# yichuan-w/LEANN

Hardware: AMD Instinct MI355X
Metric: queries/sec at recall@10>=0.9, 1M-chunk HNSW, MiniLM-L6 recompute (higher is better)
Workload: dtype fp16

## Files before the change

leann_amd/csrc/lm_attn_v2.hip:

```cpp
#include <hip/hip_fp16.h>

#include <cstdlib>

#include "lm_internal.h"

namespace lm {

typedef _Float16 half8 __attribute__((ext_vector_type(8)));
typedef _Float16 half4 __attribute__((ext_vector_type(4)));
typedef _Float16 half2v __attribute__((ext_vector_type(2)));
typedef float float16v __attribute__((ext_vector_type(16)));
typedef float float2v __attribute__((ext_vector_type(2)));

template <int NT, int HD = 32>
__global__ __launch_bounds__(256) void k_attn_varlen_hd32_v2(const __half* __restrict__ qkv, const int32_t* __restrict__ cu,
                                                             __half* __restrict__ out, int heads, float scale_log2e, int n_units) {
    extern __shared__ __align__(16) unsigned char smem[];
    const int per = gridDim.x >> 3;
    const int unit = n_units < 0 ? (int)blockIdx.x : (int)((blockIdx.x & 7) * per + (blockIdx.x >> 3));
    if (unit >= (n_units < 0 ? -n_units : n_units)) return;
    const int seq = unit / heads, h = unit % heads;
    const int tok0 = cu[seq];
    const int len = cu[seq + 1] - tok0;
    constexpr int A2_HD = HD, A2_KSTRIDE = HD + 8, PARTS = HD / 8, KS = HD / 16, DT = HD / 32;
// ... 151 lines not shown
                }
        }
    }
}

}

#ifndef LM_HOST_EMULATION
template <int HD>
static int attn_v2_launch_hd(const void* d_qkv, const int32_t* d_cu_seqlens, int32_t n_seqs, int32_t heads, int32_t max_len, void* d_out,
                             void* stream) {
    using namespace lm;
    if constexpr (HD == 32) {
        const char* gen = getenv("LEANN_MI355X_ATTN");
        const char* var = getenv("LEANN_MI355X_ATTN3");
        if (!(gen && gen[0] == '2') && !(var && var[0] == '9')) return lm_attn_v3_launch_hd32(d_qkv, d_cu_seqlens, n_seqs, heads, max_len, d_out, 0, stream);
    }
    const int nt = (max_len + 31) / 32;
    const size_t shmem = ((size_t)32 * nt * (HD + 8) + (size_t)HD * (32 * nt + 4)) * 2;
    const float scale_log2e = 1.4426950408889634f / sqrtf((float)HD);
    const char* xo = getenv("LEANN_MI355X_ATTN_XCD");
    const int n_units = (xo && xo[0] == '0') ? -(n_seqs * heads) : n_seqs * heads;
    dim3 grid((unsigned)((n_seqs * heads + 7) / 8 * 8)), block(256);
    hipStream_t st = (hipStream_t)stream;
    const __half* q = (const __half*)d_qkv;
    __half* o = (__half*)d_out;
    kt_attn_work(d_cu_seqlens, n_seqs, heads * HD, stream);
    KtScope kt(LM_KT_ATTN, stream, 0.0);
    switch (nt) {
#define CASEA(n)                                                                                                                         \
    case n: {                                                                                                                            \
// ... 46 lines not shown
```

leann_amd/csrc/lm_attn_v3.hip:

```cpp
#include <hip/hip_fp16.h>

#include <algorithm>
#include <cstdlib>

#include "lm_h384_stream.h"

namespace lm {

typedef _Float16 half2v __attribute__((ext_vector_type(2)));

__device__ __forceinline__ half4 a3_lds_read_tr16(const unsigned char* p) {
#ifdef LM_EMULATED_DEVICE
    return emul::ds_read_tr16_b64<half4>(p);
#else
    typedef __fp16 fp16x4 __attribute__((__vector_size__(4 * sizeof(__fp16))));
    typedef __attribute__((address_space(3))) fp16x4 lds_fp16x4;
    return __builtin_bit_cast(half4, __builtin_amdgcn_ds_read_tr16_b64_v4f16((lds_fp16x4*)p));
#endif
}

#if defined(LM_DIAG) && !defined(LM_EMULATED_DEVICE)
constexpr int A3_STAMP_WAVES = 1 << 17, A3_STAMP_WORDS = 12;
__device__ unsigned long long g_a3_stamps[A3_STAMP_WAVES * A3_STAMP_WORDS];
#define A3_STAMPS 1
#define A3_NOW() ((VAR & 4) ? __builtin_amdgcn_s_memtime() : 0ull)
#else
#define A3_STAMPS 0
#define A3_NOW() 0ull
#endif

__device__ __forceinline__ float a3_max3(float a, float b, float c) { return __builtin_fmaxf(__builtin_fmaxf(a, b), c); }
__device__ __forceinline__ float a3_max(float a, float b) { return __builtin_fmaxf(a, b); }

constexpr float A3_THR = 8.0f;

template <int NT, int VAR>
__global__ __launch_bounds__(256, 4) void k_attn_varlen_hd32_v3(const __half* __restrict__ qkv, const int32_t* __restrict__ cu,
                                                                __half* __restrict__ out, int heads, float scale_log2e, int n_units, int64_t hm_tokens) {
    extern __shared__ __align__(16) unsigned char smem[];
    const int per = gridDim.x >> 3;
    const int unit = n_units < 0 ? (int)blockIdx.x : (int)((blockIdx.x & 7) * per + (blockIdx.x >> 3));
    if (unit >= (n_units < 0 ? -n_units : n_units)) return;
    const int seq = unit / heads, h = unit - seq * heads;
    const int tok0 = cu[seq];
    const int len = cu[seq + 1] - tok0;
    if (len <= 0) return;
    [[maybe_unused]] const unsigned long long ts0 = A3_NOW();
    const int H = heads * 32;
    const int rsb = hm_tokens ? 64 : 6 * H;
    constexpr int Tp = 32 * NT;
    unsigned char* Ks = smem;
// ... 13 lines not shown
            const int j = wv + 4 * i;
            if (j < 2 * nt) {
                const int row = 16 * j + rl;
                const int rowc = row < len ? row : len - 1;
                const unsigned ro = (unsigned)(rowc * rsb);
                lm_dma16_sv(kbase, ro + (unsigned)((pos ^ ((row >> 2) & 3)) << 4), Ks + 1024 * j);
                lm_dma16_sv(vbase, ro + (unsigned)(pos << 4), Vs + 1024 * j);
            }
        }
    }
    half8 qraw[2][2];
#pragma unroll
    for (int qi = 0; qi < 2; ++qi) {
        const int qrow = 32 * (wv + 4 * qi) + r31;
        const unsigned char* qp = base + (int64_t)(qrow < len ? qrow : len - 1) * rsb + g * 16;
        const half8 z = {0, 0, 0, 0, 0, 0, 0, 0};
        const half8 q0 = *(const half8*)qp, q1 = *(const half8*)(qp + 32);
        qraw[qi][0] = qrow < len ? q0 : z;
        qraw[qi][1] = qrow < len ? q1 : z;
    }
    [[maybe_unused]] const unsigned long long ts1 = A3_NOW();
    T4_WAIT_VM(0);
    [[maybe_unused]] const unsigned long long ts2 = A3_NOW();
    __syncthreads();
    [[maybe_unused]] const unsigned long long ts3 = A3_NOW();
    [[maybe_unused]] unsigned long long tacc_setup = 0, tacc_loop = 0, tacc_epi = 0, nqb_done = 0;

    const int sw = (r31 >> 2) & 3;
    const unsigned char* kf0 = Ks + r31 * 64 + ((g ^ sw) << 4);
    const unsigned char* kf1 = Ks + r31 * 64 + (((2 + g) ^ sw) << 4);
    const unsigned char* vf = Vs + g * 256 + ((lane >> 2) & 3) * 64 + ((lane >> 4) & 1) * 32 + (lane & 3) * 8;
    const int tail = len & 31;
    const float lenv = (float)(tail - 4 * g);

#pragma unroll
    for (int qi = 0; qi < 2; ++qi) {
        const int qb = wv + 4 * qi;
        if (qb >= nt) break;
        const int qrow = 32 * qb + r31;
        [[maybe_unused]] const unsigned long long tq0 = A3_NOW();
        half8 qf0, qf1;
#pragma unroll
        for (int e = 0; e < 8; ++e) {
            qf0[e] = (_Float16)((float)qraw[qi][0][e] * scale_log2e);
            qf1[e] = (_Float16)((float)qraw[qi][1][e] * scale_log2e);
        }
        float16v cm, o;
#pragma unroll
        for (int r = 0; r < 16; ++r) {
            cm[r] = 0.f;
            o[r] = 0.f;
        }
        float2v l2 = {0.f, 0.f}, l2b = {0.f, 0.f};

        float16v s;
        {
            const half8 k0 = *(const half8*)kf0, k1 = *(const half8*)kf1;
            s = __builtin_amdgcn_mfma_f32_32x32x16_f16(k0, qf0, cm, 0, 0, 0);
            s = __builtin_amdgcn_mfma_f32_32x32x16_f16(k1, qf1, s, 0, 0, 0);
        }
        [[maybe_unused]] const unsigned long long tq1 = A3_NOW();
        for (int t = 0; t < nt; ++t) {
            const bool more = t + 1 < nt;
            if (t > 0) {
                const half8 k0 = *(const half8*)(kf0 + 2048 * t), k1 = *(const half8*)(kf1 + 2048 * t);
                s = __builtin_amdgcn_mfma_f32_32x32x16_f16(k0, qf0, cm, 0, 0, 0);
                s = __builtin_amdgcn_mfma_f32_32x32x16_f16(k1, qf1, s, 0, 0, 0);
            }
            const unsigned char* vt = vf + 2048 * t;
            const half4 va0 = a3_lds_read_tr16(vt), vb0 = a3_lds_read_tr16(vt + 512), va1 = a3_lds_read_tr16(vt + 1024), vb1 = a3_lds_read_tr16(vt + 1536);
            if (!more && tail) {
                float lb = (lenv - 0.5f) * 1.0e30f;
                LM_KEEP_LOCAL(lb);
#pragma unroll
                for (int r = 0; r < 16; ++r) s[r] = __builtin_amdgcn_fmed3f(s[r], lb - (float)((r & 3) + 8 * (r >> 2)) * 1.0e30f, -3.0e38f);
            }
            float tm;
            {
                const float m0 = a3_max3(s[0], s[1], s[2]), m1 = a3_max3(s[3], s[4], s[5]), m2 = a3_max3(s[6], s[7], s[8]);
                const float m3 = a3_max3(s[9], s[10], s[11]), m4 = a3_max3(s[12], s[13], s[14]);
                tm = a3_max(a3_max3(m0, m1, m2), a3_max3(m3, m4, s[15]));
                uint32_t a = __builtin_bit_cast(uint32_t, tm), b = a;
                lane32_swap(a, b);
                tm = a3_max(__builtin_bit_cast(float, a), __builtin_bit_cast(float, b));
            }
            const bool first = t == 0;
            if (first || __ballot(tm > A3_THR) != 0) {
                const float delta = first ? tm : fmaxf(tm, 0.f);
                if (!first) {
                    const float alpha = __builtin_amdgcn_exp2f(-delta);
#pragma unroll
                    for (int r = 0; r < 16; ++r) o[r] *= alpha;
                    l2 *= (float2v){alpha, alpha};
                    l2b *= (float2v){alpha, alpha};
                }
                const float2v d2 = {delta, delta};
#pragma unroll
                for (int r = 0; r < 16; r += 2) {
                    const float2v a = (float2v){s[r], s[r + 1]} - d2, b = (float2v){cm[r], cm[r + 1]} - d2;
                    s[r] = a[0];
                    s[r + 1] = a[1];
                    cm[r] = b[0];
                    cm[r + 1] = b[1];
                }
            }
            half8 p0, p1;
#pragma unroll
            for (int r = 0; r < 8; r += 2) {
                const float2v e0 = {__builtin_amdgcn_exp2f(s[r]), __builtin_amdgcn_exp2f(s[r + 1])};
                const float2v e1 = {__builtin_amdgcn_exp2f(s[8 + r]), __builtin_amdgcn_exp2f(s[9 + r])};
                l2 += e0;
                l2b += e1;
                p0[r] = (_Float16)e0[0];
                p0[r + 1] = (_Float16)e0[1];
                p1[r] = (_Float16)e1[0];
                p1[r + 1] = (_Float16)e1[1];
            }
            const half8 v0 = {va0[0], va0[1], va0[2], va0[3], vb0[0], vb0[1], vb0[2], vb0[3]};
            const half8 v1 = {va1[0], va1[1], va1[2], va1[3], vb1[0], vb1[1], vb1[2], vb1[3]};
            o = __builtin_amdgcn_mfma_f32_32x32x16_f16(v0, p0, o, 0, 0, 0);
            o = __builtin_amdgcn_mfma_f32_32x32x16_f16(v1, p1, o, 0, 0, 0);
        }
        [[maybe_unused]] const unsigned long long tq2 = A3_NOW();
        float l = (l2[0] + l2[1]) + (l2b[0] + l2b[1]);
        {
            uint32_t a = __builtin_bit_cast(uint32_t, l), b = a;
            lane32_swap(a, b);
            l = __builtin_bit_cast(float, a) + __builtin_bit_cast(float, b);
        }
        const float inv = 1.0f / l;
        if (qrow < len) {
            _Float16* orow = (_Float16*)out + (int64_t)(tok0 + qrow) * H + h * 32;
#pragma unroll
            for (int r4 = 0; r4 < 4; ++r4) {
                const float2v i2 = {inv, inv};
                const float2v a = (float2v){o[4 * r4], o[4 * r4 + 1]} * i2, b = (float2v){o[4 * r4 + 2], o[4 * r4 + 3]} * i2;
                const half4 w = {(_Float16)a[0], (_Float16)a[1], (_Float16)b[0], (_Float16)b[1]};
// ... 36 lines not shown
#if defined(LM_DIAG) && !defined(LM_HOST_EMULATION) && !defined(LM_EMULATED_DEVICE)
extern "C" int lm_attn_v3_stamps_read(unsigned long long* out, int64_t max_words, int reset) {
    const size_t total = (size_t)lm::A3_STAMP_WAVES * lm::A3_STAMP_WORDS;
    const size_t n = std::min<size_t>(total, (size_t)max_words);
    if (hipMemcpyFromSymbol(out, HIP_SYMBOL(lm::g_a3_stamps), n * sizeof(unsigned long long)) != hipSuccess) return LM_EHIP;
    if (reset) {
        void* p = nullptr;
        if (hipGetSymbolAddress(&p, HIP_SYMBOL(lm::g_a3_stamps)) != hipSuccess || hipMemset(p, 0, total * sizeof(unsigned long long)) != hipSuccess) return LM_EHIP;
    }
    return LM_OK;
}
#endif

#ifndef LM_HOST_EMULATION
int lm_attn_v3_launch_hd32(const void* d_qkv, const int32_t* d_cu_seqlens, int32_t n_seqs, int32_t heads, int32_t max_len, void* d_out, int64_t total_tokens,
                           void* stream) {
    using namespace lm;
    const int nt = (max_len + 31) / 32;
    const size_t shmem = (size_t)32 * nt * 128;
    const float scale_log2e = 1.4426950408889634f / sqrtf(32.0f);
    const char* xo = getenv("LEANN_MI355X_ATTN_XCD");
    const int n_units = (xo && xo[0] == '0') ? -(n_seqs * heads) : n_seqs * heads;
    dim3 grid((unsigned)((n_seqs * heads + 7) / 8 * 8)), block(256);
    hipStream_t st = (hipStream_t)stream;
    const __half* q = (const __half*)d_qkv;
    __half* o = (__half*)d_out;
    kt_attn_work(d_cu_seqlens, n_seqs, heads * 32, stream);
    KtScope kt(LM_KT_ATTN, stream, 0.0);
    int var = 0;
#if A3_STAMPS
    const char* ve = getenv("LEANN_MI355X_ATTN3");
    if (ve && ve[0] == '4') var = 4;
#define A3_CASE4(n) CASEV(n, 4);
#else
#define A3_CASE4(n)
#endif
    switch (nt * 8 + var) {
#define CASEV(n, v) \
    case n * 8 + v: hipLaunchKernelGGL((k_attn_varlen_hd32_v3<n, v>), grid, block, shmem, st, q, d_cu_seqlens, o, heads, scale_log2e, n_units, total_tokens); break
#define CASEA(n) CASEV(n, 0); A3_CASE4(n)
        CASEA(1); CASEA(2); CASEA(3); CASEA(4); CASEA(5); CASEA(6); CASEA(7); CASEA(8);
#undef CASEA
#undef CASEV
#undef A3_CASE4
        default: LM_FAIL(LM_EINVAL, "lm_attn_varlen_hd32_f16 supports sequence lengths 1..256");
    }
    LM_HIP(hipGetLastError());
    return LM_OK;
}
#endif
```

leann_amd/csrc/lm_encoder_forward.cpp:

```cpp
#include <algorithm>
#include <cstdint>
#include <cstdlib>
#include <string>

#include "lm_internal.h"

static int64_t small_tokens_limit() {
    const char* e = getenv("LEANN_MI355X_SMALL_TOKENS");
    return e ? (int64_t)atoll(e) : (int64_t)LM_BERT_SMALL_TOKENS;
}

lm::H384FirstHalf lm::h384_first_half_form(int32_t heads, int32_t max_len, int64_t total_tokens, int32_t n_seqs) {
    auto is = [](const char* name, char c) {
        const char* e = getenv(name);
        return e && e[0] == c;
    };
    if (heads != 12 || max_len > 256) return H384_PAIR_ROW_MAJOR;
    if (is("LEANN_MI355X_QKV_LAYOUT", '0') || is("LEANN_MI355X_ATTN3", '9') || is("LEANN_MI355X_ATTN", '2')) return H384_PAIR_ROW_MAJOR;
    if (is("LEANN_MI355X_FUSED_QKV_ATTN", '0')) return H384_PAIR_HEAD_MAJOR;
    if (is("LEANN_MI355X_FUSED_QKV_ATTN", '1')) return H384_FUSED;
    return n_seqs > 0 && total_tokens >= (int64_t)H384_FUSED_MIN_MEAN_LEN * n_seqs ? H384_FUSED : H384_PAIR_HEAD_MAJOR;
}
extern "C" int lm_h384_first_half_form(int32_t heads, int32_t max_len, int64_t total_tokens, int32_t n_seqs) {
    return (int)lm::h384_first_half_form(heads, max_len, total_tokens, n_seqs);
// ... 9 lines not shown
    if (total_tokens <= 0) return 0;
    const size_t small = total_tokens <= std::max<int64_t>(small_tokens_limit(), LM_BERT_SMALL_TOKENS) ? (size_t)total_tokens * 2560 * 2 : 0;
    return (size_t)total_tokens * (3 * 384 + 1152) * 2 + small;
}

lm::BertH384Plan lm::bert_h384_plan(const lm_bert_h384* m, int32_t n_seqs, int64_t total_tokens, int32_t max_len) {
    BertH384Plan p;
    p.small = total_tokens <= small_tokens_limit() && m->ffn % 128 == 0;
    for (int l = 0; p.small && l < m->n_layers; ++l) p.small = m->layers[l].wo && m->layers[l].w1 && m->layers[l].w2;
    p.first_half = h384_first_half_form(m->heads, max_len, total_tokens, n_seqs);
    p.qkv_gemm = !p.small && total_tokens <= qkv_gemm_tokens_limit();
    for (int l = 0; p.qkv_gemm && l < m->n_layers; ++l) p.qkv_gemm = m->layers[l].wqkv != nullptr;
    const char* f = getenv("LEANN_MI355X_FUSED_QKV_ATTN");
    if (p.qkv_gemm && f && f[0] == '1') p.qkv_gemm = false;
    else if (p.qkv_gemm) p.first_half = H384_PAIR_ROW_MAJOR;
    return p;
}

extern "C" int lm_bert_h384_forward_packed(const lm_bert_h384* m, const int32_t* d_tok, const int32_t* d_pos, const int32_t* d_cu_seqlens,
                                           int32_t n_seqs, int64_t total_tokens, int32_t max_len, void* d_workspace, size_t workspace_bytes,
                                           float* d_out, void* stream) {
    return lm::bert_h384_forward_planned(m, d_tok, d_pos, d_cu_seqlens, n_seqs, total_tokens, max_len, d_workspace, workspace_bytes, d_out, nullptr, stream);
}

int lm::bert_h384_forward_planned(const lm_bert_h384* m, const int32_t* d_tok, const int32_t* d_pos, const int32_t* d_cu_seqlens, int32_t n_seqs,
                                  int64_t total_tokens, int32_t max_len, void* d_workspace, size_t workspace_bytes, float* d_out,
                                  const BertH384Plan* plan, void* stream) {
    if (n_seqs == 0 || total_tokens == 0) return LM_OK;
    if (!m || !m->layers || !d_tok || !d_pos || !d_cu_seqlens || !d_workspace || !d_out || n_seqs < 0 || total_tokens < 0)
        LM_FAIL(LM_EINVAL, "lm_bert_h384_forward_packed: bad arguments");
// ... 18 lines not shown
    for (int l = 0; l < m->n_layers; ++l) {
        const lm_bert_h384_layer& L = m->layers[l];
        if (small) {
            if ((rc = lm_gemm_f16(x, L.wqkv, L.bqkv, nullptr, 0, 1152, 384, qkv, total_tokens, stream))) return rc;
            if ((rc = lm_attn_varlen_hd32_f16(qkv, d_cu_seqlens, n_seqs, m->heads, max_len, a, stream))) return rc;
            if ((rc = lm_gemm_f16(a, L.wo, L.bo, x, 2, 384, 384, y, total_tokens, stream))) return rc;
            if ((rc = lm_add_layernorm_f16(y, nullptr, L.ln1_gamma, L.ln1_beta, x, total_tokens, 384, m->ln_eps, stream))) return rc;
            if ((rc = lm_gemm_f16(x, L.w1, L.b1, nullptr, 1, m->ffn, 384, hid, total_tokens, stream))) return rc;
            if ((rc = lm_gemm_f16(hid, L.w2, L.b2, x, 2, 384, m->ffn, y, total_tokens, stream))) return rc;
            if ((rc = lm_add_layernorm_f16(y, nullptr, L.ln2_gamma, L.ln2_beta, x, total_tokens, 384, m->ln_eps, stream))) return rc;
            continue;
        }
        if (L.wqkv_img && first_half == H384_FUSED) {
            if ((rc = lm_qkv_attn_h384_launch(x, L.wqkv_img, L.bqkv, d_cu_seqlens, n_seqs, max_len, total_tokens, a, stream))) return rc;
        } else if (L.wqkv_img && first_half == H384_PAIR_HEAD_MAJOR) {
            if ((rc = lm_qkv_h384_launch(x, L.wqkv_img, L.bqkv, 1152, qkv, total_tokens, 1, stream))) return rc;
            if ((rc = lm_attn_v3_launch_hd32(qkv, d_cu_seqlens, n_seqs, m->heads, max_len, a, total_tokens, stream))) return rc;
        } else {
            if ((rc = qkv_gemm      ? lm_gemm_f16(x, L.wqkv, L.bqkv, nullptr, 0, 1152, 384, qkv, total_tokens, stream)
                      : L.wqkv_img ? lm_qkv_h384_f16(x, L.wqkv_img, L.bqkv, 1152, qkv, total_tokens, stream)
                                   : lm_gemm_ws_h384_f16(x, L.wqkv, L.bqkv, 1152, qkv, total_tokens, stream)))
                return rc;
            if ((rc = lm_attn_varlen_hd32_f16(qkv, d_cu_seqlens, n_seqs, m->heads, max_len, a, stream))) return rc;
        }
        if ((rc = lm_layer_tail_h384_f16(a, x, L.wo_img, L.bo, L.ln1_gamma, L.ln1_beta, m->ln_eps, L.w1_img, L.b1, L.w2_img, L.b2, L.ln2_gamma,
                                         L.ln2_beta, y, total_tokens, m->ffn, m->ln_eps, stream)))
            return rc;
        void* t = x;
        x = y;
        y = t;
    }
    return m->pooling == 1 ? lm_clspool_varlen_f16(x, d_cu_seqlens, n_seqs, 384, m->normalize, d_out, stream)
// ... 49 lines not shown
```

leann_amd/csrc/lm_h384_common.h:

```cpp
#pragma once
#include <hip/hip_fp16.h>

#include <cstring>

#include "lm_internal.h"

namespace lm {

typedef _Float16 half8 __attribute__((ext_vector_type(8)));
typedef _Float16 half4 __attribute__((ext_vector_type(4)));
typedef float float16v __attribute__((ext_vector_type(16)));
typedef float float4v __attribute__((ext_vector_type(4)));
typedef float float2v __attribute__((ext_vector_type(2)));
typedef uint32_t u32x4 __attribute__((ext_vector_type(4)));

__device__ __forceinline__ void lane32_swap(uint32_t& a, uint32_t& b) {
#ifdef LM_EMULATED_DEVICE
    const bool hi = (threadIdx.x & 63) >= 32;
    const uint32_t pa = __shfl_xor(a, 32), pb = __shfl_xor(b, 32);
    const uint32_t na = hi ? pb : a, nb = hi ? b : pa;
    a = na;
    b = nb;
#else
    auto r = __builtin_amdgcn_permlane32_swap(a, b, false, false);
    a = r[0];
    b = r[1];
#endif
}

#ifdef LM_EMULATED_DEVICE
__device__ inline void lm_dma16(const void* gsrc, unsigned char* lds_wave_base) { std::memcpy(lds_wave_base + 16 * (threadIdx.x & 63), gsrc, 16); }
__device__ inline void lm_dma16_sv(const void* sbase, unsigned voff, unsigned char* lds_wave_base) { lm_dma16((const unsigned char*)sbase + voff, lds_wave_base); }
__device__ inline void lm_dma16_sv_nt(const void* sbase, unsigned voff, unsigned char* lds_wave_base) { lm_dma16((const unsigned char*)sbase + voff, lds_wave_base); }
#else
#pragma clang diagnostic push
#pragma clang diagnostic ignored "-Winline-asm"
#ifndef LM_DMA_NOP
#define LM_DMA_NOP 3
#endif
#define LM_STR2(x) #x
#define LM_STR(x) LM_STR2(x)
#define LM_DMA_NOPS "s_nop " LM_STR(LM_DMA_NOP) "\n\t"
__device__ __forceinline__ void lm_dma16(const void* gsrc, unsigned char* lds_wave_base) {
// ... 82 lines not shown
```

leann_amd/csrc/lm_internal.h:

```cpp
#pragma once
#include <hip/hip_runtime.h>

#include <cstdint>
#include <cstdio>
#include <string>
#include <vector>

#include "../../include/leann_mi355x.h"

namespace lm {

void set_error(const std::string& msg);

#define LM_HIP(expr)                                                                       \
    do {                                                                                   \
        hipError_t _e = (expr);                                                            \
        if (_e != hipSuccess) {                                                            \
            lm::set_error(std::string(#expr) + ": " + hipGetErrorString(_e));              \
            return LM_EHIP;                                                                \
        }                                                                                  \
    } while (0)

#ifndef LM_KEEP_LOCAL
#define LM_KEEP_LOCAL(v) asm volatile("" : "+v"(v))
// ... 89 lines not shown
struct lm_recompute;
namespace lm {
int rc_prepare(lm_recompute* rc, const int32_t* d_ids, const unsigned long long* d_n, int64_t cap, unsigned long long* d_total,
               unsigned long long* d_maxlen, unsigned long long* d_split, hipStream_t st);
void rc_prepared(lm_recompute* rc, const int32_t* d_ids, int32_t n, int64_t total, int32_t max_len, const unsigned long long* split);
int32_t rc_width(const lm_recompute* rc);
inline bool bert_h384_envelope_ok(int n_layers, int heads, int ffn) { return n_layers > 0 && heads * 32 == 384 && ffn >= 192 && ffn <= 1728 && ffn % 192 == 0; }
#define LM_BERT_H384_ENVELOPE_TEXT "hidden 384 = heads x 32 and ffn a multiple of 192 in [192, 1728]"
enum H384FirstHalf : int { H384_FUSED = 0, H384_PAIR_HEAD_MAJOR = 1, H384_PAIR_ROW_MAJOR = 2 };
constexpr int H384_FUSED_MIN_MEAN_LEN = 216;
H384FirstHalf h384_first_half_form(int32_t heads, int32_t max_len, int64_t total_tokens, int32_t n_seqs);
struct BertH384Plan {
    bool small = false;
    bool qkv_gemm = false;
    H384FirstHalf first_half = H384_PAIR_HEAD_MAJOR;
};
BertH384Plan bert_h384_plan(const lm_bert_h384* m, int32_t n_seqs, int64_t total_tokens, int32_t max_len);
int bert_h384_forward_planned(const lm_bert_h384* m, const int32_t* d_tok, const int32_t* d_pos, const int32_t* d_cu_seqlens, int32_t n_seqs,
                              int64_t total_tokens, int32_t max_len, void* d_workspace, size_t workspace_bytes, float* d_out, const BertH384Plan* plan,
                              void* stream);

}

int lm_qkv_h384_launch(const void* d_x, const void* d_w_img, const float* d_bias, int32_t n_out, void* d_out, int64_t tokens, int32_t head_major, void* stream);

int lm_attn_v3_launch_hd32(const void* d_qkv, const int32_t* d_cu_seqlens, int32_t n_seqs, int32_t heads, int32_t max_len, void* d_out, int64_t total_tokens,
                           void* stream);

int lm_qkv_attn_h384_launch(const void* d_x, const void* d_wqkv_img, const float* d_bqkv, const int32_t* d_cu_seqlens, int32_t n_seqs, int32_t max_len,
                            int64_t total_tokens, void* d_out, void* stream);

int lm_add_layernorm_r16_launch(const void* d_x, const void* d_residual, const void* d_gamma, const void* d_beta, void* d_out,
                                int64_t rows, int32_t hidden, float eps, void* stream);
```

leann_amd/csrc/lm_qkv_h384.hip:

```cpp
#include <cstdlib>
#include <cstring>
#include <utility>

#include "lm_h384_stream.h"

namespace lm {

typedef _Float16 qk_half2 __attribute__((ext_vector_type(2)));

constexpr int QK_STAGES = 4;
constexpr int QK_TILE_OFF = QK_STAGES * T4_SLAB;
constexpr int QK_TILE = 4096;
constexpr int QK_BIAS_OFF = QK_TILE_OFF + 8 * QK_TILE;

struct QkAddr {
    const unsigned char* a1[2][8];
};
template <int ST, int KS>
__device__ __forceinline__ half8 qk_frag(const QkAddr& c) {
    return *(const half8*)(c.a1[ST >> 1][KS & 7] + (ST & 1) * T4_SLAB + 256 * (KS >> 3));
}

template <int RD>
struct QkCarry {
    half8 ring[RD];
    float16v biasv;
};

template <int STEP, bool ODD>
__device__ __forceinline__ void qk_epilogue_step(const float16v& a, const float16v& b, unsigned char* tile, __half* __restrict__ out, int64_t tok0,
                                                 int rows_valid, int N, int feat0, int r31, int g, int lane) {
    if constexpr (STEP < 4) {
        constexpr int q = STEP;
        const float2v v0 = (float2v){a[4 * q], a[4 * q + 1]} + (float2v){b[4 * q], b[4 * q + 1]};
        const float2v v1 = (float2v){a[4 * q + 2], a[4 * q + 3]} + (float2v){b[4 * q + 2], b[4 * q + 3]};
        const qk_half2 h0 = __builtin_convertvector(v0, qk_half2), h1 = __builtin_convertvector(v1, qk_half2);
        const half4 y = {h0[0], h0[1], h1[0], h1[1]};
        *(half4*)(tile + r31 * 128 + ((((ODD ? 4 : 0) + q) ^ (r31 & 7)) << 4) + 8 * g) = y;
    } else if constexpr (ODD && STEP == 4) {
        LM_WAVE_SYNC();
    } else if constexpr (ODD && (STEP == 5 || STEP == 6)) {
        if (rows_valid > 0) {
#pragma unroll
            for (int jj = 0; jj < 2; ++jj) {
                const int id = 64 * (2 * (STEP - 5) + jj) + lane, c16 = id & 7;
                const int row = (id >> 3) < rows_valid ? (id >> 3) : rows_valid - 1;
                const u32x4 v = *(const u32x4*)(tile + row * 128 + ((c16 ^ (row & 7)) << 4));
                const int64_t off = N > 0 ? ((tok0 + row) * N + feat0) * 2 + 16 * c16
                                          : (((int64_t)(feat0 >> 5) + (c16 >> 2)) * (int64_t)(-N) + tok0 + row) * 64 + 16 * (c16 & 3);
                *(u32x4*)((unsigned char*)out + off) = v;
            }
        }
    }
}

template <int ST, int P, bool NEXT, bool PREV, bool DMA, int RD, int I>
__device__ __forceinline__ void qk_slot(const QkAddr& c, const float* bs_next, const half8 (&xf)[ML_KS], float16v (&acc)[2][2], QkCarry<RD>& cy,
                                        unsigned char* tile, __half* __restrict__ out, int64_t tok0, int rows_valid, int N, int feat0_prev, int r31, int g,
                                        int lane, const unsigned char* dsrc, unsigned voff, unsigned char* ddst) {
    if constexpr (I == 24 - RD && NEXT) {
        if (rows_valid > 0) t4_wait_vm<DMA ? (P == 0 ? 14 : 10) : 0>();
        else t4_wait_vm<DMA ? 6 : 0>();
        T4_BARRIER();
    }
    if constexpr (I == 0) acc[P][0] = __builtin_amdgcn_mfma_f32_32x32x16_f16(cy.ring[0], xf[0], cy.biasv, 0, 0, 0);
    else if constexpr (I == 1) {
        const float16v z = {0.f, 0.f, 0.f, 0.f, 0.f, 0.f, 0.f, 0.f, 0.f, 0.f, 0.f, 0.f, 0.f, 0.f, 0.f, 0.f};
        acc[P][1] = __builtin_amdgcn_mfma_f32_32x32x16_f16(cy.ring[1 % RD], xf[1], z, 0, 0, 0);
    } else acc[P][I & 1] = __builtin_amdgcn_mfma_f32_32x32x16_f16(cy.ring[I % RD], xf[I], acc[P][I & 1], 0, 0, 0);
    if constexpr (I + RD < 24) cy.ring[I % RD] = qk_frag<ST, I + RD>(c);
    else if constexpr (NEXT) cy.ring[I % RD] = qk_frag<(ST + 1) % QK_STAGES, I + RD - 24>(c);
    if constexpr (NEXT && I >= 16 && I < 20) {
        constexpr int q = I - 16;
        const float4v bv = *(const float4v*)(bs_next + 8 * q);
#pragma unroll
        for (int i = 0; i < 4; ++i) cy.biasv[4 * q + i] = bv[i];
    }
    if constexpr (DMA && I == 1) t4_dma_group<3>(dsrc, voff, ddst);
    if constexpr (PREV && I >= 3 && I <= 15 && (I & 1)) {
        constexpr bool ODD = (P ^ 1) != 0;
        qk_epilogue_step<(I - 3) / 2, ODD>(acc[P ^ 1][0], acc[P ^ 1][1], tile, out, tok0, rows_valid, N, feat0_prev, r31, g, lane);
    }
    __builtin_amdgcn_sched_barrier(0);
}
template <int ST, int P, bool NEXT, bool PREV, bool DMA, int RD, int... I>
__device__ __forceinline__ void qk_slots(std::integer_sequence<int, I...>, const QkAddr& c, const float* bs_next, const half8 (&xf)[ML_KS],
                                         float16v (&acc)[2][2], QkCarry<RD>& cy, unsigned char* tile, __half* __restrict__ out, int64_t tok0, int rows_valid,
                                         int N, int feat0_prev, int r31, int g, int lane, const unsigned char* dsrc, unsigned voff, unsigned char* ddst) {
    (qk_slot<ST, P, NEXT, PREV, DMA, RD, I>(c, bs_next, xf, acc, cy, tile, out, tok0, rows_valid, N, feat0_prev, r31, g, lane, dsrc, voff, ddst), ...);
}

template <int RD>
__global__ __launch_bounds__(512) LM_TWO_WAVES_PER_SIMD void k_qkv_h384(const __half* __restrict__ x, const __half* __restrict__ w_img,
                                                                         const float* __restrict__ bias, __half* __restrict__ out, int T, int Nfeat,
                                                                         int head_major) {
    extern __shared__ __align__(16) unsigned char smem[];
    float* bss = (float*)(smem + QK_BIAS_OFF);
    const int N = Nfeat;
    const int Nst = head_major ? -T : Nfeat;
    const int tid = threadIdx.x, lane = tid & 63;
#ifdef LM_EMULATED_DEVICE
    const int wv = tid >> 6;
#else
    const int wv = __builtin_amdgcn_readfirstlane(tid >> 6);
#endif
    const int r31 = lane & 31, g = lane >> 5;
    const int64_t tok0 = (int64_t)blockIdx.x * 256 + wv * 32;
    const int rows_valid = (int)(T - tok0 < 32 ? (T - tok0 > 0 ? T - tok0 : 0) : 32);
    const int nslab = N >> 5;
    const unsigned char* gw = (const unsigned char*)w_img;
    const unsigned voff0 = (unsigned)lane * 16u;
    unsigned char* tile = smem + QK_TILE_OFF + wv * QK_TILE;
    auto dma_slab = [&](int s, int st) {
        const int sl = s < nslab ? s : nslab - 1;
// ... 22 lines not shown
        ad.a1[1][k7] = smem + 2 * T4_SLAB + a;
    }
    T4_WAIT_VM(0);
    __syncthreads();
    const float* bl = bss + 4 * g;
    float16v acc[2][2];
    QkCarry<RD> cy;
#pragma unroll
    for (int q = 0; q < 4; ++q) {
        const float4v bv = *(const float4v*)(bl + 8 * q);
#pragma unroll
        for (int i = 0; i < 4; ++i) cy.biasv[4 * q + i] = bv[i];
    }
#pragma unroll
    for (int i = 0; i < RD; ++i) cy.ring[i] = *(const half8*)(ad.a1[0][i & 7] + 256 * (i >> 3));
#define QK_SLAB(ST, P, NEXT, PREV, S)                                                                                                          \
    qk_slots<ST, P, NEXT, PREV, NEXT, RD>(std::make_integer_sequence<int, 24>{}, ad, bl + 32 * ((S) + 1), xf, acc, cy, tile, out, tok0, rows_valid, Nst, \
                                          32 * ((S) - 2), r31, g, lane, gw + (int64_t)((S) + 3 < nslab ? (S) + 3 : nslab - 1) * T4_SLAB + 3072 * wv, voff0, \
                                          smem + (((ST) + 3) % QK_STAGES) * T4_SLAB + 3072 * wv)
    QK_SLAB(0, 0, true, false, 0);
    for (int s = 1; s + 3 < nslab; s += 4) {
        QK_SLAB(1, 1, true, true, s);
        QK_SLAB(2, 0, true, true, s + 1);
        QK_SLAB(3, 1, true, true, s + 2);
        QK_SLAB(0, 0, true, true, s + 3);
    }
    {
        const int s = nslab - 3;
        QK_SLAB(1, 1, true, true, s);
        QK_SLAB(2, 0, true, true, s + 1);
        qk_slots<3, 1, false, true, false, RD>(std::make_integer_sequence<int, 24>{}, ad, nullptr, xf, acc, cy, tile, out, tok0, rows_valid, Nst, 32 * (s + 2 - 2),
                                               r31, g, lane, nullptr, voff0, nullptr);
    }
#undef QK_SLAB
    {
        const int f0 = 32 * (nslab - 2);
        qk_epilogue_step<0, true>(acc[1][0], acc[1][1], tile, out, tok0, rows_valid, Nst, f0, r31, g, lane);
        qk_epilogue_step<1, true>(acc[1][0], acc[1][1], tile, out, tok0, rows_valid, Nst, f0, r31, g, lane);
        qk_epilogue_step<2, true>(acc[1][0], acc[1][1], tile, out, tok0, rows_valid, Nst, f0, r31, g, lane);
        qk_epilogue_step<3, true>(acc[1][0], acc[1][1], tile, out, tok0, rows_valid, Nst, f0, r31, g, lane);
        qk_epilogue_step<4, true>(acc[1][0], acc[1][1], tile, out, tok0, rows_valid, Nst, f0, r31, g, lane);
        qk_epilogue_step<5, true>(acc[1][0], acc[1][1], tile, out, tok0, rows_valid, Nst, f0, r31, g, lane);
        qk_epilogue_step<6, true>(acc[1][0], acc[1][1], tile, out, tok0, rows_valid, Nst, f0, r31, g, lane);
    }
    T4_WAIT_VM(0);
}

}


int lm_qkv_h384_launch(const void* d_x, const void* d_w_img, const float* d_bias, int32_t n_out, void* d_out, int64_t tokens, int32_t head_major, void* stream) {
    using namespace lm;
    if (tokens == 0) return LM_OK;
    if (!d_x || !d_w_img || !d_bias || !d_out || tokens < 0 || tokens > 0x7fffffff) LM_FAIL(LM_EINVAL, "bad linear arguments");
    if (n_out < 256 || n_out % 128 || n_out > 6144) LM_FAIL(LM_EINVAL, "lm_qkv_h384_f16: n_out must be a multiple of 128 in [256, 6144]");
    const size_t shmem = (size_t)QK_BIAS_OFF + (size_t)n_out * 4;
    KtScope kt(LM_KT_QKV, stream, 2.0 * (double)tokens * n_out * ML_H);
    static DynLdsAttr attr;
    LM_HIP(ensure_dyn_lds(attr, (const void*)k_qkv_h384<4>, shmem));
    hipLaunchKernelGGL(k_qkv_h384<4>, dim3((unsigned)((tokens + 255) / 256)), dim3(512), shmem, (hipStream_t)stream, (const __half*)d_x, (const __half*)d_w_img,
                       d_bias, (__half*)d_out, (int)tokens, n_out, (int)(head_major != 0));
    LM_HIP(hipGetLastError());
    return LM_OK;
}

extern "C" int lm_qkv_h384_f16(const void* d_x, const void* d_w_img, const float* d_bias, int32_t n_out, void* d_out, int64_t tokens, void* stream) {
    return lm_qkv_h384_launch(d_x, d_w_img, d_bias, n_out, d_out, tokens, 0, stream);
}
```

Baseline: 679.8.

## Fold attention Q prescale into QKV GEMM epilogue and peel first softmax tile

```diff
diff --git a/leann_amd/csrc/lm_attn_v2.hip b/leann_amd/csrc/lm_attn_v2.hip
--- a/leann_amd/csrc/lm_attn_v2.hip
+++ b/leann_amd/csrc/lm_attn_v2.hip
@@ -189,7 +189,7 @@
     if constexpr (HD == 32) {
         const char* gen = getenv("LEANN_MI355X_ATTN");
         const char* var = getenv("LEANN_MI355X_ATTN3");
-        if (!(gen && gen[0] == '2') && !(var && var[0] == '9')) return lm_attn_v3_launch_hd32(d_qkv, d_cu_seqlens, n_seqs, heads, max_len, d_out, 0, stream);
+        if (!(gen && gen[0] == '2') && !(var && var[0] == '9')) return lm_attn_v3_launch_hd32(d_qkv, d_cu_seqlens, n_seqs, heads, max_len, d_out, 0, 0, stream);
     }
     const int nt = (max_len + 31) / 32;
     const size_t shmem = ((size_t)32 * nt * (HD + 8) + (size_t)HD * (32 * nt + 4)) * 2;
diff --git a/leann_amd/csrc/lm_attn_v3.hip b/leann_amd/csrc/lm_attn_v3.hip
--- a/leann_amd/csrc/lm_attn_v3.hip
+++ b/leann_amd/csrc/lm_attn_v3.hip
@@ -2,6 +2,7 @@
 
 #include <algorithm>
 #include <cstdlib>
+#include <type_traits>
 
 #include "lm_h384_stream.h"
 
@@ -34,7 +35,7 @@
 
 constexpr float A3_THR = 8.0f;
 
-template <int NT, int VAR>
+template <int NT, int VAR, int PQ = 0>
 __global__ __launch_bounds__(256, 4) void k_attn_varlen_hd32_v3(const __half* __restrict__ qkv, const int32_t* __restrict__ cu,
                                                                 __half* __restrict__ out, int heads, float scale_log2e, int n_units, int64_t hm_tokens) {
     extern __shared__ __align__(16) unsigned char smem[];
@@ -78,10 +79,15 @@
     for (int qi = 0; qi < 2; ++qi) {
         const int qrow = 32 * (wv + 4 * qi) + r31;
         const unsigned char* qp = base + (int64_t)(qrow < len ? qrow : len - 1) * rsb + g * 16;
-        const half8 z = {0, 0, 0, 0, 0, 0, 0, 0};
         const half8 q0 = *(const half8*)qp, q1 = *(const half8*)(qp + 32);
-        qraw[qi][0] = qrow < len ? q0 : z;
-        qraw[qi][1] = qrow < len ? q1 : z;
+        if constexpr (PQ) {
+            qraw[qi][0] = q0;
+            qraw[qi][1] = q1;
+        } else {
+            const half8 z = {0, 0, 0, 0, 0, 0, 0, 0};
+            qraw[qi][0] = qrow < len ? q0 : z;
+            qraw[qi][1] = qrow < len ? q1 : z;
+        }
     }
     [[maybe_unused]] const unsigned long long ts1 = A3_NOW();
     T4_WAIT_VM(0);
@@ -104,31 +110,29 @@
         const int qrow = 32 * qb + r31;
         [[maybe_unused]] const unsigned long long tq0 = A3_NOW();
         half8 qf0, qf1;
-#pragma unroll
-        for (int e = 0; e < 8; ++e) {
-            qf0[e] = (_Float16)((float)qraw[qi][0][e] * scale_log2e);
-            qf1[e] = (_Float16)((float)qraw[qi][1][e] * scale_log2e);
+        if constexpr (PQ) {
+            qf0 = qraw[qi][0];
+            qf1 = qraw[qi][1];
+        } else {
+#pragma unroll
+            for (int e = 0; e < 8; ++e) {
+                qf0[e] = lm_q_prescale(qraw[qi][0][e], scale_log2e);
+                qf1[e] = lm_q_prescale(qraw[qi][1][e], scale_log2e);
+            }
         }
         float16v cm, o;
-#pragma unroll
-        for (int r = 0; r < 16; ++r) {
-            cm[r] = 0.f;
-            o[r] = 0.f;
-        }
-        float2v l2 = {0.f, 0.f}, l2b = {0.f, 0.f};
-
-        float16v s;
-        {
-            const half8 k0 = *(const half8*)kf0, k1 = *(const half8*)kf1;
-            s = __builtin_amdgcn_mfma_f32_32x32x16_f16(k0, qf0, cm, 0, 0, 0);
-            s = __builtin_amdgcn_mfma_f32_32x32x16_f16(k1, qf1, s, 0, 0, 0);
-        }
+        float2v l2, l2b;
         [[maybe_unused]] const unsigned long long tq1 = A3_NOW();
-        for (int t = 0; t < nt; ++t) {
+
+        auto tile = [&](auto first_c, const int t) __attribute__((always_inline)) {
+            constexpr bool FIRST = decltype(first_c)::value;
+            const float16v zero = {0.f, 0.f, 0.f, 0.f, 0.f, 0.f, 0.f, 0.f, 0.f, 0.f, 0.f, 0.f, 0.f, 0.f, 0.f, 0.f};
             const bool more = t + 1 < nt;
-            if (t > 0) {
+            float16v s;
+            {
                 const half8 k0 = *(const half8*)(kf0 + 2048 * t), k1 = *(const half8*)(kf1 + 2048 * t);
-                s = __builtin_amdgcn_mfma_f32_32x32x16_f16(k0, qf0, cm, 0, 0, 0);
+                if constexpr (FIRST) s = __builtin_amdgcn_mfma_f32_32x32x16_f16(k0, qf0, zero, 0, 0, 0);
+                else s = __builtin_amdgcn_mfma_f32_32x32x16_f16(k0, qf0, cm, 0, 0, 0);
                 s = __builtin_amdgcn_mfma_f32_32x32x16_f16(k1, qf1, s, 0, 0, 0);
             }
             const unsigned char* vt = vf + 2048 * t;
@@ -148,16 +152,24 @@
                 lane32_swap(a, b);
                 tm = a3_max(__builtin_bit_cast(float, a), __builtin_bit_cast(float, b));
             }
-            const bool first = t == 0;
-            if (first || __ballot(tm > A3_THR) != 0) {
-                const float delta = first ? tm : fmaxf(tm, 0.f);
-                if (!first) {
-                    const float alpha = __builtin_amdgcn_exp2f(-delta);
-#pragma unroll
-                    for (int r = 0; r < 16; ++r) o[r] *= alpha;
-                    l2 *= (float2v){alpha, alpha};
-                    l2b *= (float2v){alpha, alpha};
+            if constexpr (FIRST) {
+                const float2v d2 = {tm, tm};
+                const float nm = 0.f - tm;
+#pragma unroll
+                for (int r = 0; r < 16; r += 2) {
+                    const float2v a = (float2v){s[r], s[r + 1]} - d2;
+                    s[r] = a[0];
+                    s[r + 1] = a[1];
+                    cm[r] = nm;
+                    cm[r + 1] = nm;
                 }
+            } else if (__ballot(tm > A3_THR) != 0) {
+                const float delta = fmaxf(tm, 0.f);
+                const float alpha = __builtin_amdgcn_exp2f(-delta);
+#pragma unroll
+                for (int r = 0; r < 16; ++r) o[r] *= alpha;
+                l2 *= (float2v){alpha, alpha};
+                l2b *= (float2v){alpha, alpha};
                 const float2v d2 = {delta, delta};
 #pragma unroll
                 for (int r = 0; r < 16; r += 2) {
@@ -173,8 +185,13 @@
             for (int r = 0; r < 8; r += 2) {
                 const float2v e0 = {__builtin_amdgcn_exp2f(s[r]), __builtin_amdgcn_exp2f(s[r + 1])};
                 const float2v e1 = {__builtin_amdgcn_exp2f(s[8 + r]), __builtin_amdgcn_exp2f(s[9 + r])};
-                l2 += e0;
-                l2b += e1;
+                if (FIRST && r == 0) {
+                    l2 = e0;
+                    l2b = e1;
+                } else {
+                    l2 += e0;
+                    l2b += e1;
+                }
                 p0[r] = (_Float16)e0[0];
                 p0[r + 1] = (_Float16)e0[1];
                 p1[r] = (_Float16)e1[0];
@@ -182,9 +199,12 @@
             }
             const half8 v0 = {va0[0], va0[1], va0[2], va0[3], vb0[0], vb0[1], vb0[2], vb0[3]};
             const half8 v1 = {va1[0], va1[1], va1[2], va1[3], vb1[0], vb1[1], vb1[2], vb1[3]};
-            o = __builtin_amdgcn_mfma_f32_32x32x16_f16(v0, p0, o, 0, 0, 0);
+            if constexpr (FIRST) o = __builtin_amdgcn_mfma_f32_32x32x16_f16(v0, p0, zero, 0, 0, 0);
+            else o = __builtin_amdgcn_mfma_f32_32x32x16_f16(v0, p0, o, 0, 0, 0);
             o = __builtin_amdgcn_mfma_f32_32x32x16_f16(v1, p1, o, 0, 0, 0);
-        }
+        };
+        tile(std::true_type{}, 0);
+        for (int t = 1; t < nt; ++t) tile(std::false_type{}, t);
         [[maybe_unused]] const unsigned long long tq2 = A3_NOW();
         float l = (l2[0] + l2[1]) + (l2b[0] + l2b[1]);
         {
@@ -251,11 +271,12 @@
 
 #ifndef LM_HOST_EMULATION
 int lm_attn_v3_launch_hd32(const void* d_qkv, const int32_t* d_cu_seqlens, int32_t n_seqs, int32_t heads, int32_t max_len, void* d_out, int64_t total_tokens,
-                           void* stream) {
+                           int32_t q_prescaled, void* stream) {
     using namespace lm;
+    if (q_prescaled && total_tokens <= 0) LM_FAIL(LM_EINVAL, "lm_attn_v3: prescaled Q comes with the head-major layout only");
     const int nt = (max_len + 31) / 32;
     const size_t shmem = (size_t)32 * nt * 128;
-    const float scale_log2e = 1.4426950408889634f / sqrtf(32.0f);
+    const float scale_log2e = attn_scale_log2e_hd32();
     const char* xo = getenv("LEANN_MI355X_ATTN_XCD");
     const int n_units = (xo && xo[0] == '0') ? -(n_seqs * heads) : n_seqs * heads;
     dim3 grid((unsigned)((n_seqs * heads + 7) / 8 * 8)), block(256);
@@ -274,7 +295,10 @@
 #endif
     switch (nt * 8 + var) {
 #define CASEV(n, v) \
-    case n * 8 + v: hipLaunchKernelGGL((k_attn_varlen_hd32_v3<n, v>), grid, block, shmem, st, q, d_cu_seqlens, o, heads, scale_log2e, n_units, total_tokens); break
+    case n * 8 + v:                                                                                                                                           \
+        if (q_prescaled) hipLaunchKernelGGL((k_attn_varlen_hd32_v3<n, v, 1>), grid, block, shmem, st, q, d_cu_seqlens, o, heads, scale_log2e, n_units, total_tokens); \
+        else hipLaunchKernelGGL((k_attn_varlen_hd32_v3<n, v, 0>), grid, block, shmem, st, q, d_cu_seqlens, o, heads, scale_log2e, n_units, total_tokens);           \
+        break
 #define CASEA(n) CASEV(n, 0); A3_CASE4(n)
         CASEA(1); CASEA(2); CASEA(3); CASEA(4); CASEA(5); CASEA(6); CASEA(7); CASEA(8);
 #undef CASEA
diff --git a/leann_amd/csrc/lm_encoder_forward.cpp b/leann_amd/csrc/lm_encoder_forward.cpp
--- a/leann_amd/csrc/lm_encoder_forward.cpp
+++ b/leann_amd/csrc/lm_encoder_forward.cpp
@@ -47,6 +47,8 @@
     const char* f = getenv("LEANN_MI355X_FUSED_QKV_ATTN");
     if (p.qkv_gemm && f && f[0] == '1') p.qkv_gemm = false;
     else if (p.qkv_gemm) p.first_half = H384_PAIR_ROW_MAJOR;
+    const char* pq = getenv("LEANN_MI355X_QKV_PRESCALED_Q");
+    p.q_prescaled = p.first_half == H384_PAIR_HEAD_MAJOR && !(pq && pq[0] == '0');
     return p;
 }
 
@@ -95,8 +97,8 @@
         if (L.wqkv_img && first_half == H384_FUSED) {
             if ((rc = lm_qkv_attn_h384_launch(x, L.wqkv_img, L.bqkv, d_cu_seqlens, n_seqs, max_len, total_tokens, a, stream))) return rc;
         } else if (L.wqkv_img && first_half == H384_PAIR_HEAD_MAJOR) {
-            if ((rc = lm_qkv_h384_launch(x, L.wqkv_img, L.bqkv, 1152, qkv, total_tokens, 1, stream))) return rc;
-            if ((rc = lm_attn_v3_launch_hd32(qkv, d_cu_seqlens, n_seqs, m->heads, max_len, a, total_tokens, stream))) return rc;
+            if ((rc = lm_qkv_h384_launch(x, L.wqkv_img, L.bqkv, 1152, qkv, total_tokens, pl.q_prescaled ? 2 : 1, stream))) return rc;
+            if ((rc = lm_attn_v3_launch_hd32(qkv, d_cu_seqlens, n_seqs, m->heads, max_len, a, total_tokens, pl.q_prescaled, stream))) return rc;
         } else {
             if ((rc = qkv_gemm      ? lm_gemm_f16(x, L.wqkv, L.bqkv, nullptr, 0, 1152, 384, qkv, total_tokens, stream)
                       : L.wqkv_img ? lm_qkv_h384_f16(x, L.wqkv_img, L.bqkv, 1152, qkv, total_tokens, stream)
diff --git a/leann_amd/csrc/lm_h384_common.h b/leann_amd/csrc/lm_h384_common.h
--- a/leann_amd/csrc/lm_h384_common.h
+++ b/leann_amd/csrc/lm_h384_common.h
@@ -27,6 +27,8 @@
     b = r[1];
 #endif
 }
+
+__device__ __forceinline__ _Float16 lm_q_prescale(_Float16 q, float c) { return (_Float16)((float)q * c); }
 
 #ifdef LM_EMULATED_DEVICE
 __device__ inline void lm_dma16(const void* gsrc, unsigned char* lds_wave_base) { std::memcpy(lds_wave_base + 16 * (threadIdx.x & 63), gsrc, 16); }
diff --git a/leann_amd/csrc/lm_internal.h b/leann_amd/csrc/lm_internal.h
--- a/leann_amd/csrc/lm_internal.h
+++ b/leann_amd/csrc/lm_internal.h
@@ -1,6 +1,7 @@
 #pragma once
 #include <hip/hip_runtime.h>
 
+#include <cmath>
 #include <cstdint>
 #include <cstdio>
 #include <string>
@@ -127,7 +128,9 @@
     bool small = false;
     bool qkv_gemm = false;
     H384FirstHalf first_half = H384_PAIR_HEAD_MAJOR;
+    bool q_prescaled = true;
 };
+inline float attn_scale_log2e_hd32() { return 1.4426950408889634f / sqrtf(32.0f); }
 BertH384Plan bert_h384_plan(const lm_bert_h384* m, int32_t n_seqs, int64_t total_tokens, int32_t max_len);
 int bert_h384_forward_planned(const lm_bert_h384* m, const int32_t* d_tok, const int32_t* d_pos, const int32_t* d_cu_seqlens, int32_t n_seqs,
                               int64_t total_tokens, int32_t max_len, void* d_workspace, size_t workspace_bytes, float* d_out, const BertH384Plan* plan,
@@ -138,7 +141,7 @@
 int lm_qkv_h384_launch(const void* d_x, const void* d_w_img, const float* d_bias, int32_t n_out, void* d_out, int64_t tokens, int32_t head_major, void* stream);
 
 int lm_attn_v3_launch_hd32(const void* d_qkv, const int32_t* d_cu_seqlens, int32_t n_seqs, int32_t heads, int32_t max_len, void* d_out, int64_t total_tokens,
-                           void* stream);
+                           int32_t q_prescaled, void* stream);
 
 int lm_qkv_attn_h384_launch(const void* d_x, const void* d_wqkv_img, const float* d_bqkv, const int32_t* d_cu_seqlens, int32_t n_seqs, int32_t max_len,
                             int64_t total_tokens, void* d_out, void* stream);
diff --git a/leann_amd/csrc/lm_qkv_h384.hip b/leann_amd/csrc/lm_qkv_h384.hip
--- a/leann_amd/csrc/lm_qkv_h384.hip
+++ b/leann_amd/csrc/lm_qkv_h384.hip
@@ -27,15 +27,19 @@
     float16v biasv;
 };
 
-template <int STEP, bool ODD>
+template <int STEP, bool ODD, bool QS>
 __device__ __forceinline__ void qk_epilogue_step(const float16v& a, const float16v& b, unsigned char* tile, __half* __restrict__ out, int64_t tok0,
-                                                 int rows_valid, int N, int feat0, int r31, int g, int lane) {
+                                                 int rows_valid, int N, int feat0, int r31, int g, int lane, float qc) {
     if constexpr (STEP < 4) {
         constexpr int q = STEP;
         const float2v v0 = (float2v){a[4 * q], a[4 * q + 1]} + (float2v){b[4 * q], b[4 * q + 1]};
         const float2v v1 = (float2v){a[4 * q + 2], a[4 * q + 3]} + (float2v){b[4 * q + 2], b[4 * q + 3]};
         const qk_half2 h0 = __builtin_convertvector(v0, qk_half2), h1 = __builtin_convertvector(v1, qk_half2);
-        const half4 y = {h0[0], h0[1], h1[0], h1[1]};
+        half4 y = {h0[0], h0[1], h1[0], h1[1]};
+        if constexpr (QS) {
+#pragma unroll
+            for (int i = 0; i < 4; ++i) y[i] = lm_q_prescale(y[i], qc);
+        }
         *(half4*)(tile + r31 * 128 + ((((ODD ? 4 : 0) + q) ^ (r31 & 7)) << 4) + 8 * g) = y;
     } else if constexpr (ODD && STEP == 4) {
         LM_WAVE_SYNC();
@@ -54,10 +58,10 @@
     }
 }
 
-template <int ST, int P, bool NEXT, bool PREV, bool DMA, int RD, int I>
+template <int ST, int P, bool NEXT, bool PREV, bool DMA, int RD, bool QS, int I>
 __device__ __forceinline__ void qk_slot(const QkAddr& c, const float* bs_next, const half8 (&xf)[ML_KS], float16v (&acc)[2][2], QkCarry<RD>& cy,
                                         unsigned char* tile, __half* __restrict__ out, int64_t tok0, int rows_valid, int N, int feat0_prev, int r31, int g,
-                                        int lane, const unsigned char* dsrc, unsigned voff, unsigned char* ddst) {
+                                        int lane, const unsigned char* dsrc, unsigned voff, unsigned char* ddst, float qc) {
     if constexpr (I == 24 - RD && NEXT) {
         if (rows_valid > 0) t4_wait_vm<DMA ? (P == 0 ? 14 : 10) : 0>();
         else t4_wait_vm<DMA ? 6 : 0>();
@@ -79,25 +83,27 @@
     if constexpr (DMA && I == 1) t4_dma_group<3>(dsrc, voff, ddst);
     if constexpr (PREV && I >= 3 && I <= 15 && (I & 1)) {
         constexpr bool ODD = (P ^ 1) != 0;
-        qk_epilogue_step<(I - 3) / 2, ODD>(acc[P ^ 1][0], acc[P ^ 1][1], tile, out, tok0, rows_valid, N, feat0_prev, r31, g, lane);
+        qk_epilogue_step<(I - 3) / 2, ODD, QS>(acc[P ^ 1][0], acc[P ^ 1][1], tile, out, tok0, rows_valid, N, feat0_prev, r31, g, lane, qc);
     }
     __builtin_amdgcn_sched_barrier(0);
 }
-template <int ST, int P, bool NEXT, bool PREV, bool DMA, int RD, int... I>
+template <int ST, int P, bool NEXT, bool PREV, bool DMA, int RD, bool QS, int... I>
 __device__ __forceinline__ void qk_slots(std::integer_sequence<int, I...>, const QkAddr& c, const float* bs_next, const half8 (&xf)[ML_KS],
                                          float16v (&acc)[2][2], QkCarry<RD>& cy, unsigned char* tile, __half* __restrict__ out, int64_t tok0, int rows_valid,
-                                         int N, int feat0_prev, int r31, int g, int lane, const unsigned char* dsrc, unsigned voff, unsigned char* ddst) {
-    (qk_slot<ST, P, NEXT, PREV, DMA, RD, I>(c, bs_next, xf, acc, cy, tile, out, tok0, rows_valid, N, feat0_prev, r31, g, lane, dsrc, voff, ddst), ...);
-}
-
-template <int RD>
+                                         int N, int feat0_prev, int r31, int g, int lane, const unsigned char* dsrc, unsigned voff, unsigned char* ddst,
+                                         float qc) {
+    (qk_slot<ST, P, NEXT, PREV, DMA, RD, QS, I>(c, bs_next, xf, acc, cy, tile, out, tok0, rows_valid, N, feat0_prev, r31, g, lane, dsrc, voff, ddst, qc), ...);
+}
+
+template <int RD, int QSLABS = 0>
 __global__ __launch_bounds__(512) LM_TWO_WAVES_PER_SIMD void k_qkv_h384(const __half* __restrict__ x, const __half* __restrict__ w_img,
                                                                          const float* __restrict__ bias, __half* __restrict__ out, int T, int Nfeat,
-                                                                         int head_major) {
+                                                                         int head_major, float q_scale) {
     extern __shared__ __align__(16) unsigned char smem[];
     float* bss = (float*)(smem + QK_BIAS_OFF);
     const int N = Nfeat;
     const int Nst = head_major ? -T : Nfeat;
+    if constexpr (QSLABS > 0) __builtin_assume(Nst < 0);
     const int tid = threadIdx.x, lane = tid & 63;
 #ifdef LM_EMULATED_DEVICE
     const int wv = tid >> 6;
@@ -150,34 +156,43 @@
     }
 #pragma unroll
     for (int i = 0; i < RD; ++i) cy.ring[i] = *(const half8*)(ad.a1[0][i & 7] + 256 * (i >> 3));
-#define QK_SLAB(ST, P, NEXT, PREV, S)                                                                                                          \
-    qk_slots<ST, P, NEXT, PREV, NEXT, RD>(std::make_integer_sequence<int, 24>{}, ad, bl + 32 * ((S) + 1), xf, acc, cy, tile, out, tok0, rows_valid, Nst, \
+#define QK_SLAB(ST, P, NEXT, PREV, S, QS)                                                                                                      \
+    qk_slots<ST, P, NEXT, PREV, NEXT, RD, QS>(std::make_integer_sequence<int, 24>{}, ad, bl + 32 * ((S) + 1), xf, acc, cy, tile, out, tok0, rows_valid, Nst, \
                                           32 * ((S) - 2), r31, g, lane, gw + (int64_t)((S) + 3 < nslab ? (S) + 3 : nslab - 1) * T4_SLAB + 3072 * wv, voff0, \
-                                          smem + (((ST) + 3) % QK_STAGES) * T4_SLAB + 3072 * wv)
-    QK_SLAB(0, 0, true, false, 0);
-    for (int s = 1; s + 3 < nslab; s += 4) {
-        QK_SLAB(1, 1, true, true, s);
-        QK_SLAB(2, 0, true, true, s + 1);
-        QK_SLAB(3, 1, true, true, s + 2);
-        QK_SLAB(0, 0, true, true, s + 3);
+                                          smem + (((ST) + 3) % QK_STAGES) * T4_SLAB + 3072 * wv, q_scale)
+    static_assert(QSLABS % 4 == 0, "the Q slabs end with an iteration of the slab loop");
+    QK_SLAB(0, 0, true, false, 0, false);
+    int s4 = 1;
+    if constexpr (QSLABS > 0)
+        for (; s4 < QSLABS; s4 += 4) {
+            QK_SLAB(1, 1, true, true, s4, true);
+            QK_SLAB(2, 0, true, true, s4 + 1, true);
+            QK_SLAB(3, 1, true, true, s4 + 2, true);
+            QK_SLAB(0, 0, true, true, s4 + 3, true);
+        }
+    for (int s = s4; s + 3 < nslab; s += 4) {
+        QK_SLAB(1, 1, true, true, s, false);
+        QK_SLAB(2, 0, true, true, s + 1, false);
+        QK_SLAB(3, 1, true, true, s + 2, false);
+        QK_SLAB(0, 0, true, true, s + 3, false);
     }
     {
         const int s = nslab - 3;
-        QK_SLAB(1, 1, true, true, s);
-        QK_SLAB(2, 0, true, true, s + 1);
-        qk_slots<3, 1, false, true, false, RD>(std::make_integer_sequence<int, 24>{}, ad, nullptr, xf, acc, cy, tile, out, tok0, rows_valid, Nst, 32 * (s + 2 - 2),
-                                               r31, g, lane, nullptr, voff0, nullptr);
+        QK_SLAB(1, 1, true, true, s, false);
+        QK_SLAB(2, 0, true, true, s + 1, false);
+        qk_slots<3, 1, false, true, false, RD, false>(std::make_integer_sequence<int, 24>{}, ad, nullptr, xf, acc, cy, tile, out, tok0, rows_valid, Nst, 32 * (s + 2 - 2),
+                                               r31, g, lane, nullptr, voff0, nullptr, q_scale);
     }
 #undef QK_SLAB
     {
         const int f0 = 32 * (nslab - 2);
-        qk_epilogue_step<0, true>(acc[1][0], acc[1][1], tile, out, tok0, rows_valid, Nst, f0, r31, g, lane);
-        qk_epilogue_step<1, true>(acc[1][0], acc[1][1], tile, out, tok0, rows_valid, Nst, f0, r31, g, lane);
-        qk_epilogue_step<2, true>(acc[1][0], acc[1][1], tile, out, tok0, rows_valid, Nst, f0, r31, g, lane);
-        qk_epilogue_step<3, true>(acc[1][0], acc[1][1], tile, out, tok0, rows_valid, Nst, f0, r31, g, lane);
-        qk_epilogue_step<4, true>(acc[1][0], acc[1][1], tile, out, tok0, rows_valid, Nst, f0, r31, g, lane);
-        qk_epilogue_step<5, true>(acc[1][0], acc[1][1], tile, out, tok0, rows_valid, Nst, f0, r31, g, lane);
-        qk_epilogue_step<6, true>(acc[1][0], acc[1][1], tile, out, tok0, rows_valid, Nst, f0, r31, g, lane);
+        qk_epilogue_step<0, true, false>(acc[1][0], acc[1][1], tile, out, tok0, rows_valid, Nst, f0, r31, g, lane, q_scale);
+        qk_epilogue_step<1, true, false>(acc[1][0], acc[1][1], tile, out, tok0, rows_valid, Nst, f0, r31, g, lane, q_scale);
+        qk_epilogue_step<2, true, false>(acc[1][0], acc[1][1], tile, out, tok0, rows_valid, Nst, f0, r31, g, lane, q_scale);
+        qk_epilogue_step<3, true, false>(acc[1][0], acc[1][1], tile, out, tok0, rows_valid, Nst, f0, r31, g, lane, q_scale);
+        qk_epilogue_step<4, true, false>(acc[1][0], acc[1][1], tile, out, tok0, rows_valid, Nst, f0, r31, g, lane, q_scale);
+        qk_epilogue_step<5, true, false>(acc[1][0], acc[1][1], tile, out, tok0, rows_valid, Nst, f0, r31, g, lane, q_scale);
+        qk_epilogue_step<6, true, false>(acc[1][0], acc[1][1], tile, out, tok0, rows_valid, Nst, f0, r31, g, lane, q_scale);
     }
     T4_WAIT_VM(0);
 }
@@ -190,12 +205,20 @@
     if (tokens == 0) return LM_OK;
     if (!d_x || !d_w_img || !d_bias || !d_out || tokens < 0 || tokens > 0x7fffffff) LM_FAIL(LM_EINVAL, "bad linear arguments");
     if (n_out < 256 || n_out % 128 || n_out > 6144) LM_FAIL(LM_EINVAL, "lm_qkv_h384_f16: n_out must be a multiple of 128 in [256, 6144]");
+    if (head_major == 2 && n_out != 1152) LM_FAIL(LM_EINVAL, "lm_qkv_h384: prescaled Q needs n_out 1152 (Q, K, V of 12 heads x 32)");
     const size_t shmem = (size_t)QK_BIAS_OFF + (size_t)n_out * 4;
     KtScope kt(LM_KT_QKV, stream, 2.0 * (double)tokens * n_out * ML_H);
-    static DynLdsAttr attr;
-    LM_HIP(ensure_dyn_lds(attr, (const void*)k_qkv_h384<4>, shmem));
-    hipLaunchKernelGGL(k_qkv_h384<4>, dim3((unsigned)((tokens + 255) / 256)), dim3(512), shmem, (hipStream_t)stream, (const __half*)d_x, (const __half*)d_w_img,
-                       d_bias, (__half*)d_out, (int)tokens, n_out, (int)(head_major != 0));
+    static DynLdsAttr attr, attr_pq;
+    const dim3 grid((unsigned)((tokens + 255) / 256));
+    if (head_major == 2) {
+        LM_HIP(ensure_dyn_lds(attr_pq, (const void*)k_qkv_h384<4, 12>, shmem));
+        hipLaunchKernelGGL((k_qkv_h384<4, 12>), grid, dim3(512), shmem, (hipStream_t)stream, (const __half*)d_x, (const __half*)d_w_img, d_bias, (__half*)d_out,
+                           (int)tokens, n_out, 1, attn_scale_log2e_hd32());
+    } else {
+        LM_HIP(ensure_dyn_lds(attr, (const void*)k_qkv_h384<4>, shmem));
+        hipLaunchKernelGGL((k_qkv_h384<4>), grid, dim3(512), shmem, (hipStream_t)stream, (const __half*)d_x, (const __half*)d_w_img, d_bias, (__half*)d_out,
+                           (int)tokens, n_out, (int)(head_major != 0), 0.f);
+    }
     LM_HIP(hipGetLastError());
     return LM_OK;
 }
```

Result: no change. 683.5, median of 2 (+0.5%).
